# OpenPPL/ppq

Hardware: AMD Instinct MI355X
Metric: calibration samples/sec (RuntimeCalibrationPass, KL 2048-bin, ResNet-50 INT8) (higher is better)
Workload: dtype f32; 1 GPU; ResNet-50 topology (53 Conv + 1 Gemm, BN folded, seeded He init), RuntimeCalibrationPass kl 2048 bins, per-tensor INT8 activations, per-channel INT8 weights, 279 batches x 32 x 3x224x224 per GPU; samples=8928, batch=32, observed_tensors=72, rccl_ranks=1, async_observe=False, cache_params=False, channels_last=False, fuse_params=True, batch_observations=True, reuse_activations=False, replayed_batches=0, hip_graph=auto, graph_replays=0, miopen_find=False

## Files before the change

### ppq_amd/csrc/pointwise_conv.hip

```cpp
#include "common.hpp"
#include "epilogue_sinks.hpp"
#include "job_table.hpp"

namespace ppqhip {
namespace {

typedef float f32x16 __attribute__((ext_vector_type(16)));

struct PwArgs {
    const float* x; const float* w; const float* bias; float* y;
    uint32_t c, o, q;
    uint32_t in_plane, out_plane;
    uint32_t in_w, stride;
    uint32_t tiles_m;
    FastDiv div_plane, div_wo, div_tiles_m;
};

template <int WM, int WN, int TM, int TN, int BK, bool VEC>
__global__ __launch_bounds__(256) void conv1x1_kernel(const PwArgs g) {
    static_assert(WM * WN == 4 && (BK == 16 || BK == 32), "4 waves; BK 16 or 32");
    constexpr int BM = WM * TM * 32, BN = WN * TN * 32, RS = BK + 4, HK = BK / 2, LW = VEC ? 4 : 1;
    constexpr int WL = BM * BK / (256 * LW), XL = BK * BN / (256 * LW);
    constexpr int WROWS = 256 * LW / BK, XROWS = 256 * LW / BN;
    static_assert(BN / LW <= 256 && WL >= 1 && XL >= 1, "tile too small / too wide for the loader");
    typedef float ldv __attribute__((ext_vector_type(LW)));
    __shared__ __attribute__((aligned(16))) float Ws[2][BM * RS];
    __shared__ __attribute__((aligned(16))) float Xs[2][BK * BN];

    const uint32_t t = threadIdx.x, lane = t & 63u, wave = t >> 6;
    const uint32_t tq = fdiv(blockIdx.x, g.div_tiles_m), tm = blockIdx.x - tq * g.tiles_m;
    const uint32_t m0 = tm * BM, q0 = tq * BN;

    const uint32_t wk = (t % (BK / LW)) * LW, wm = t / (BK / LW);
    const uint32_t xc = (t % (BN / LW)) * LW, xk = t / (BN / LW);
    uint32_t woff[WL], xoff;
#pragma unroll
    for (int r = 0; r < WL; r++) woff[r] = min(m0 + wm + WROWS * r, g.o - 1u) * g.c + wk;
    {
        const uint32_t qx = min(q0 + xc, g.q - LW);
        const uint32_t img = fdiv(qx, g.div_plane), p = qx - img * g.out_plane;
        uint32_t src = p;
        if (g.stride != 1u) { const uint32_t oh = fdiv(p, g.div_wo), ow = p - oh * g.div_wo.d; src = (oh * g.in_w + ow) * g.stride; }
        xoff = img * g.c * g.in_plane + src + xk * g.in_plane;
    }
    const uint32_t xstep = XROWS * g.in_plane;
    ldv wr[WL], xr[XL];
    auto load_tile = [&](uint32_t k0) {
        if (k0 + BK <= g.c) {
#pragma unroll
            for (int r = 0; r < WL; r++) wr[r] = *reinterpret_cast<const ldv*>(g.w + (woff[r] + k0));
            const float* xp = g.x + (xoff + k0 * g.in_plane);
#pragma unroll
            for (int r = 0; r < XL; r++) xr[r] = *reinterpret_cast<const ldv*>(xp + r * xstep);
        } else {
#pragma unroll
            for (int r = 0; r < WL; r++) {
                ldv pad = -0.0f;
                wr[r] = (k0 + wk < g.c) ? *reinterpret_cast<const ldv*>(g.w + (woff[r] + k0)) : pad;
            }
#pragma unroll
            for (int r = 0; r < XL; r++) {
                ldv pad = 0.0f;
                xr[r] = (k0 + xk + XROWS * r < g.c) ? *reinterpret_cast<const ldv*>(g.x + (xoff + k0 * g.in_plane + r * xstep)) : pad;
            }
        }
    };
    auto store_tile = [&](int buf) {
#pragma unroll
        for (int r = 0; r < WL; r++) {
            float* row = &Ws[buf][(wm + WROWS * r) * RS];
            if constexpr (VEC) {
                *reinterpret_cast<float2*>(row + (wk >> 1)) = make_float2(wr[r][0], wr[r][2]);
                *reinterpret_cast<float2*>(row + HK + (wk >> 1)) = make_float2(wr[r][1], wr[r][3]);
            } else {
                row[(wk & 1u) * HK + (wk >> 1)] = wr[r][0];
            }
        }
#pragma unroll
        for (int r = 0; r < XL; r++) *reinterpret_cast<ldv*>(&Xs[buf][(xk + XROWS * r) * BN + xc]) = xr[r];
    };

    const uint32_t i = lane & 31u, h = lane >> 5;
    const uint32_t row0 = (wave / WN) * (TM * 32), col0 = (wave % WN) * (TN * 32);
    f32x16 acc[TM][TN];
#pragma unroll
    for (int mt = 0; mt < TM; mt++)
#pragma unroll
        for (int nt = 0; nt < TN; nt++)
#pragma unroll
            for (int r = 0; r < 16; r++) acc[mt][nt][r] = 0.0f;

    const uint32_t tiles_k = (g.c + BK - 1) / BK;
    load_tile(0);
    store_tile(0);
    __syncthreads();
    for (uint32_t kt = 0; kt < tiles_k; kt++) {
        const int buf = (int)(kt & 1u);
        const bool more = kt + 1 < tiles_k;
        if (more) load_tile((kt + 1) * BK);
        const float* ws = &Ws[buf][(row0 + i) * RS + h * HK];
        const float* xs = &Xs[buf][h * BN + col0 + i];
        float a[TM][HK];
#pragma unroll
        for (int mt = 0; mt < TM; mt++)
#pragma unroll
            for (int v = 0; v < HK / 4; v++) {
                const float4 f = *reinterpret_cast<const float4*>(ws + mt * 32 * RS + 4 * v);
                a[mt][4 * v] = f.x; a[mt][4 * v + 1] = f.y; a[mt][4 * v + 2] = f.z; a[mt][4 * v + 3] = f.w;
            }
#pragma unroll
        for (int s = 0; s < HK; s++) {
            float b[TN];
#pragma unroll
            for (int nt = 0; nt < TN; nt++) b[nt] = xs[2 * s * BN + nt * 32];
#pragma unroll
            for (int mt = 0; mt < TM; mt++)
#pragma unroll
                for (int nt = 0; nt < TN; nt++)
                    acc[mt][nt] = __builtin_amdgcn_mfma_f32_32x32x2f32(a[mt][s], b[nt], acc[mt][nt], 0, 0, 0);
        }
        if (more) store_tile(buf ^ 1);
        __syncthreads();
    }

    const bool has_bias = g.bias != nullptr;
    float bv[TM][16];
#pragma unroll
    for (int mt = 0; mt < TM; mt++)
#pragma unroll
        for (int r = 0; r < 16; r++)
            bv[mt][r] = has_bias ? g.bias[min(m0 + row0 + mt * 32 + (r & 3) + 8 * (r >> 2) + 4 * h, g.o - 1u)] : 0.0f;
#pragma unroll
    for (int nt = 0; nt < TN; nt++) {
        const uint32_t qc = q0 + col0 + nt * 32 + i;
        if (qc >= g.q) continue;
        const uint32_t img = fdiv(qc, g.div_plane), p = qc - img * g.out_plane;
        float* yc = g.y + (img * g.o * g.out_plane + p);
#pragma unroll
        for (int mt = 0; mt < TM; mt++)
#pragma unroll
            for (int r = 0; r < 16; r++) {
                const uint32_t row = m0 + row0 + mt * 32 + (r & 3) + 8 * (r >> 2) + 4 * h;
                if (row >= g.o) continue;
                float v = acc[mt][nt][r];
                if (has_bias) v = v + bv[mt][r];
                yc[row * g.out_plane] = v;
            }
    }
}

constexpr int kWM = 2, kWN = 2, kTM = 1, kTN = 1, kBK = 32;

inline bool aligned4(const void* p) { return (reinterpret_cast<uintptr_t>(p) & 3u) == 0; }

struct PwEpArgs {
    const float* bias_b; const float* resid;
    uint32_t tiles, relu;
};

template <int WM, int WN, int BK, bool VEC, int FORM, class SINKS>
__global__ __launch_bounds__(WM * WN * 64, (WM * WN * 64 * kEpStatWgPerCu + 255) / 256)
void conv1x1_epilogue_kernel(const PwArgs g, const PwEpArgs e, const typename SINKS::Args sk) {
    static_assert(BK == 16 || BK == 32, "BK 16 or 32");
    constexpr int NT = WM * WN * 64;
    constexpr bool RESID = FORM != 0, BIAS_B = FORM == 1;
    constexpr int BM = WM * 32, BN = WN * 32, RS = BK + 4, HK = BK / 2, LW = VEC ? 4 : 1;
    constexpr int WL = BM * BK / (NT * LW), XL = BK * BN / (NT * LW);
    constexpr int WROWS = NT * LW / BK, XROWS = NT * LW / BN;
    static_assert(BN / LW <= NT && WL >= 1 && XL >= 1, "tile too small / too wide for the loader");
    typedef float ldv __attribute__((ext_vector_type(LW)));
    __shared__ __attribute__((aligned(16))) float Ws[2][BM * RS];
    __shared__ __attribute__((aligned(16))) float Xs[2][BK * BN];
    __shared__ float Bs[2][2 * BM];
    extern __shared__ int sink_lds[];

    const uint32_t t = threadIdx.x, lane = t & 63u, wave = t >> 6;
    uint32_t tile, tile_end;
    even_split(e.tiles, gridDim.x, blockIdx.x, tile, tile_end);
    SINKS sinks;
    sinks.init(sk, sink_lds);

    const uint32_t wk = (t % (BK / LW)) * LW, wm = t / (BK / LW);
    const uint32_t xc = (t % (BN / LW)) * LW, xk = t / (BN / LW);
    const uint32_t xstep = XROWS * g.in_plane;
    uint32_t m0, q0, woff[WL], xoff;
    float bpre = 0.0f;
    int par = 0;
    auto setup = [&](uint32_t ti) {
        const uint32_t tq = fdiv(ti, g.div_tiles_m), tm = ti - tq * g.tiles_m;
        m0 = tm * BM; q0 = tq * BN;
#pragma unroll
        for (int r = 0; r < WL; r++) woff[r] = min(m0 + wm + WROWS * r, g.o - 1u) * g.c + wk;
        const uint32_t qx = min(q0 + xc, g.q - LW);
        const uint32_t img = fdiv(qx, g.div_plane), p = qx - img * g.out_plane;
        uint32_t src = p;
        if (g.stride != 1u) { const uint32_t oh = fdiv(p, g.div_wo), ow = p - oh * g.div_wo.d; src = (oh * g.in_w + ow) * g.stride; }
        xoff = img * g.c * g.in_plane + src + xk * g.in_plane;
        if (t < 2 * BM) {
            const uint32_t row = min(m0 + (t & (BM - 1)), g.o - 1u);
            bpre = t < BM ? g.bias[row] : (BIAS_B ? e.bias_b[row] : 0.0f);
        }
    };
    ldv wr[WL], xr[XL];
    auto load_tile = [&](uint32_t k0) {
        if (k0 + BK <= g.c) {
#pragma unroll
            for (int r = 0; r < WL; r++) wr[r] = *reinterpret_cast<const ldv*>(g.w + (woff[r] + k0));
            const float* xp = g.x + (xoff + k0 * g.in_plane);
#pragma unroll
            for (int r = 0; r < XL; r++) xr[r] = *reinterpret_cast<const ldv*>(xp + r * xstep);
        } else {
#pragma unroll
            for (int r = 0; r < WL; r++) {
                ldv pad = -0.0f;
                wr[r] = (k0 + wk < g.c) ? *reinterpret_cast<const ldv*>(g.w + (woff[r] + k0)) : pad;
            }
#pragma unroll
            for (int r = 0; r < XL; r++) {
                ldv pad = 0.0f;
                xr[r] = (k0 + xk + XROWS * r < g.c) ? *reinterpret_cast<const ldv*>(g.x + (xoff + k0 * g.in_plane + r * xstep)) : pad;
            }
        }
    };
    auto store_tile = [&](int buf) {
#pragma unroll
        for (int r = 0; r < WL; r++) {
            float* row = &Ws[buf][(wm + WROWS * r) * RS];
            if constexpr (VEC) {
                *reinterpret_cast<float2*>(row + (wk >> 1)) = make_float2(wr[r][0], wr[r][2]);
                *reinterpret_cast<float2*>(row + HK + (wk >> 1)) = make_float2(wr[r][1], wr[r][3]);
            } else {
                row[(wk & 1u) * HK + (wk >> 1)] = wr[r][0];
            }
        }
#pragma unroll
        for (int r = 0; r < XL; r++) *reinterpret_cast<ldv*>(&Xs[buf][(xk + XROWS * r) * BN + xc]) = xr[r];
    };

    const uint32_t i = lane & 31u, h = lane >> 5;
    const uint32_t row0 = (wave / WN) * 32, col0 = (wave % WN) * 32;
    const uint32_t tiles_k = (g.c + BK - 1) / BK;
    const bool relu = e.relu != 0;

    setup(tile);
    load_tile(0);
    sinks.begin();
    for (;;) {
        const uint32_t em0 = m0, eq0 = q0;
        const uint32_t qc = eq0 + col0 + i, rbase = em0 + row0 + 4 * h;
        const bool col_in = qc < g.q;
        const uint32_t qcl = min(qc, g.q - 1u);
        const uint32_t img = fdiv(qcl, g.div_plane), p = qcl - img * g.out_plane;
        const uint32_t ycol = img * g.o * g.out_plane + p;
        f32x16 acc;
#pragma unroll
        for (int r = 0; r < 16; r++) acc[r] = 0.0f;

        auto multiply = [&](int buf) {
            const float* ws = &Ws[buf][(row0 + i) * RS + h * HK];
            const float* xs = &Xs[buf][h * BN + col0 + i];
            float a[HK];
#pragma unroll
            for (int v = 0; v < HK / 4; v++) {
                const float4 f = *reinterpret_cast<const float4*>(ws + 4 * v);
                a[4 * v] = f.x; a[4 * v + 1] = f.y; a[4 * v + 2] = f.z; a[4 * v + 3] = f.w;
            }
#pragma unroll
            for (int s = 0; s < HK; s++) acc = __builtin_amdgcn_mfma_f32_32x32x2f32(a[s], xs[2 * s * BN], acc, 0, 0, 0);
        };
        store_tile(0);
        if (t < 2 * BM) Bs[par][t] = bpre;
        __syncthreads();
        for (uint32_t kt = 0; kt + 1 < tiles_k; kt++) {
            const int buf = (int)(kt & 1u);
            load_tile((kt + 1) * BK);
            multiply(buf);
            store_tile(buf ^ 1);
            __syncthreads();
        }
        float rv[16];
#pragma unroll
        for (int r = 0; r < 16; r++)
            rv[r] = RESID ? e.resid[ycol + min(rbase + (r & 3) + 8 * (r >> 2), g.o - 1u) * g.out_plane] : 0.0f;
        multiply((int)((tiles_k - 1) & 1u));
        __syncthreads();

        const bool next = tile + 1 < tile_end;
        const bool full = em0 + BM <= g.o && eq0 + BN <= g.q;
        const float* bs = &Bs[par][row0 + 4 * h];
#pragma unroll
        for (int j = 0; j < 4; j++) {
            if (j == 2 && next) { setup(tile + 1); load_tile(0); }
            float va[4], vb[4], vo[4], ba[4], bb[4];
#pragma unroll
            for (int u = 0; u < 4; u++) { ba[u] = bs[8 * j + u]; bb[u] = BIAS_B ? bs[BM + 8 * j + u] : 0.0f; }
#pragma unroll
            for (int u = 0; u < 4; u++) {
                const int r = 4 * j + u;
                const float xa = acc[r] + ba[u];
                if (!RESID) { va[u] = act(xa, relu); vb[u] = 0.0f; vo[u] = 0.0f; continue; }
                va[u] = xa;
                float rr = rv[r];
                if (BIAS_B) rr = rr + bb[u];
                vb[u] = rr;
                vo[u] = act(xa + rr, relu);
            }
#pragma unroll
            for (int u = 0; u < 4; u++) {
                const uint32_t row = rbase + u + 8 * j;
                if (col_in && row < g.o) g.y[ycol + min(row, g.o - 1u) * g.out_plane] = RESID ? vo[u] : va[u];
            }
            if (full) {
                EpStored<float4> s4{};
                s4.a = make_float4(va[0], va[1], va[2], va[3]);
                if (BIAS_B) s4.b = make_float4(vb[0], vb[1], vb[2], vb[3]);
                if (RESID) s4.out = make_float4(vo[0], vo[1], vo[2], vo[3]);
                sinks.template feed4<true>(s4, true, j == 0);
            } else {
#pragma unroll
                for (int u = 0; u < 4; u++) {
                    EpStored<float> s1{};
                    s1.a = va[u]; s1.b = vb[u]; s1.out = vo[u];
                    sinks.feed1(s1, col_in && rbase + u + 8 * j < g.o);
                }
            }
            __builtin_amdgcn_sched_barrier(0);
        }
        if (!next) break;
        tile++;
        par ^= 1;
    }
    sinks.finish(sk, blockIdx.x, sink_lds);
}

constexpr int kFWM = 2, kFWN = 4;
static_assert(kFWM * kFWN * 64 == kEpStatBlock, "the fused launch has the sink launches' workgroup");

template <int FORM, class SINKS>
void launch_fused(bool vec, uint32_t grid, uint32_t lds_bytes, hipStream_t s, const PwArgs& g, const PwEpArgs& e,
                  const typename SINKS::Args& sk) {
    if (vec) hipLaunchKernelGGL((conv1x1_epilogue_kernel<kFWM, kFWN, kBK, true, FORM, SINKS>), dim3(grid), dim3(kEpStatBlock), lds_bytes, s, g, e, sk);
    else hipLaunchKernelGGL((conv1x1_epilogue_kernel<kFWM, kFWN, kBK, false, FORM, SINKS>), dim3(grid), dim3(kEpStatBlock), lds_bytes, s, g, e, sk);
}

template <int FORM>
void launch_fused_hist(bool vec, uint32_t grid, hipStream_t s, const PwArgs& g, const PwEpArgs& e, const EpHistSinks& sk, int asym, int clip) {
    constexpr bool R = FORM != 0, B = FORM == 1;
    const uint32_t lds = sk.lds_ints * (uint32_t)sizeof(int);
    switch ((asym ? 2 : 0) | (clip ? 1 : 0)) {
        case 0: launch_fused<FORM, EpHistSet<R, B, false, false, kEpStatBlock, !R>>(vec, grid, lds, s, g, e, sk); break;
        case 1: launch_fused<FORM, EpHistSet<R, B, false, true, kEpStatBlock, !R>>(vec, grid, lds, s, g, e, sk); break;
        case 2: launch_fused<FORM, EpHistSet<R, B, true, false, kEpStatBlock, !R>>(vec, grid, lds, s, g, e, sk); break;
        default: launch_fused<FORM, EpHistSet<R, B, true, true, kEpStatBlock, !R>>(vec, grid, lds, s, g, e, sk); break;
    }
}

int refuse(const char* what, const char* why) {
    set_error("%s: %s", what, why);
    return PPQHIP_ERR_INVALID_VALUE;
}

}
}

using namespace ppqhip;

extern "C" int ppqhip_conv1x1(const float* x, const float* w, const float* bias, float* y, int64_t n, int64_t c, int64_t h, int64_t wd,
                              int64_t o, int64_t stride, void* stream) {
    const char* what = "conv1x1";
    constexpr int64_t kMax = 2147483647;
    if (n < 0 || c <= 0 || h <= 0 || wd <= 0 || o <= 0) { set_error("%s: non-positive size", what); return PPQHIP_ERR_INVALID_VALUE; }
    if (stride != 1 && stride != 2) { set_error("%s: stride must be 1 or 2", what); return PPQHIP_ERR_UNSUPPORTED; }
    if (n == 0) return PPQHIP_OK;
    if (x == nullptr || w == nullptr || y == nullptr) { set_error("%s: null pointer", what); return PPQHIP_ERR_INVALID_VALUE; }
    const int64_t ho = (h - 1) / stride + 1, wo = (wd - 1) / stride + 1;
    if (n > kMax || c > kMax || h > kMax || wd > kMax || o > kMax || (double)n * (double)c * (double)h * (double)wd > (double)kMax
        || (double)n * (double)o * (double)ho * (double)wo > (double)kMax || (double)o * (double)c > (double)kMax) {
        set_error("%s: more than 2^31 - 1 elements in x, w or y", what); return PPQHIP_ERR_INVALID_VALUE;
    }
    std::vector<Span> ins, outs;
    ins.push_back(span_of(x, n * c * h * wd)); ins.push_back(span_of(w, o * c));
    if (bias != nullptr) ins.push_back(span_of(bias, o));
    outs.push_back(span_of(y, n * o * ho * wo));
    if (int st = check_overlap(what, ins, outs)) return st;
    if (!aligned4(x) || !aligned4(w) || !aligned4(y) || !aligned4(bias)) return PPQHIP_NOT_FUSED;

    PwArgs g;
    g.x = x; g.w = w; g.bias = bias; g.y = y;
    g.c = (uint32_t)c; g.o = (uint32_t)o; g.q = (uint32_t)(n * ho * wo);
    g.in_plane = (uint32_t)(h * wd); g.out_plane = (uint32_t)(ho * wo); g.in_w = (uint32_t)wd; g.stride = (uint32_t)stride;
    g.div_plane = make_fastdiv(g.out_plane); g.div_wo = make_fastdiv((uint32_t)wo);
    hipStream_t s = (hipStream_t)stream;
    const bool vec = stride == 1 && g.out_plane % 4u == 0 && c % 4 == 0 && aligned16(x) && aligned16(w);
    constexpr uint32_t BM = kWM * kTM * 32, BN = kWN * kTN * 32;
    g.tiles_m = (g.o + BM - 1) / BM;
    g.div_tiles_m = make_fastdiv(g.tiles_m);
    const dim3 grid(g.tiles_m * ((g.q + BN - 1) / BN));
    if (vec) hipLaunchKernelGGL((conv1x1_kernel<kWM, kWN, kTM, kTN, kBK, true>), grid, dim3(256), 0, s, g);
    else hipLaunchKernelGGL((conv1x1_kernel<kWM, kWN, kTM, kTN, kBK, false>), grid, dim3(256), 0, s, g);
    return finish_launch(what);
}

extern "C" int ppqhip_conv1x1_epilogue(const float* x, const float* w, const float* bias_a, const float* resid, const float* bias_b,
                                       float* out, int64_t n, int64_t c, int64_t h, int64_t wd, int64_t o, int64_t stride, int relu,
                                       int sink_kind, void* dst_a, void* dst_r, void* dst_out, float p0_a, float p1_a, float p0_r,
                                       float p1_r, float p0_out, float p1_out, int64_t num_bins, int asymmetric, int clip_outliers,
                                       int64_t max_workgroups, void* stream) {
    const char* what = "conv1x1_epilogue";
    constexpr int64_t kMax = 2147483647;
    if (n < 0 || c <= 0 || h <= 0 || wd <= 0 || o <= 0) return refuse(what, "non-positive size");
    if (stride != 1 && stride != 2) { set_error("%s: stride must be 1 or 2", what); return PPQHIP_ERR_UNSUPPORTED; }
    if (max_workgroups < 0) return refuse(what, "max_workgroups is negative");
    if (sink_kind != PPQHIP_SINK_NONE && sink_kind != PPQHIP_SINK_MINMAX && sink_kind != PPQHIP_SINK_HIST)
        return refuse(what, "unknown sink kind");
    if (n == 0) return PPQHIP_OK;
    if (x == nullptr || w == nullptr || bias_a == nullptr || out == nullptr) return refuse(what, "null pointer");
    if (resid == nullptr && bias_b != nullptr) return refuse(what, "bias_b without a residual");
    const int64_t ho = (h - 1) / stride + 1, wo = (wd - 1) / stride + 1;
    if (n > kMax || c > kMax || h > kMax || wd > kMax || o > kMax || (double)n * (double)c * (double)h * (double)wd > (double)kMax
        || (double)n * (double)o * (double)ho * (double)wo > (double)kMax || (double)o * (double)c > (double)kMax)
        return refuse(what, "more than 2^31 - 1 elements in x, w or out");
    if (resid == nullptr && (dst_a != nullptr || dst_r != nullptr)) return refuse(what, "without a residual only out has a sink");
    if (bias_b == nullptr && dst_r != nullptr) return refuse(what, "without bias_b, the residual is only read: it has no sink");
    const bool hist = sink_kind == PPQHIP_SINK_HIST, minmax = sink_kind == PPQHIP_SINK_MINMAX;
    if (hist && (num_bins <= 0 || num_bins > kMax)) return refuse(what, "histogram is empty or too large");
    if ((dst_a && (dst_a == dst_r || dst_a == dst_out)) || (dst_r && dst_r == dst_out)) return refuse(what, "two sinks share one accumulator");
    const int64_t ny = n * o * ho * wo;
    std::vector<Span> ins, outs;
    ins.push_back(span_of(x, n * c * h * wd)); ins.push_back(span_of(w, o * c)); ins.push_back(span_of(bias_a, o));
    if (resid != nullptr) ins.push_back(span_of(resid, ny));
    if (bias_b != nullptr) ins.push_back(span_of(bias_b, o));
    outs.push_back(span_of(out, ny));
    if (int st = check_overlap(what, ins, outs)) return st;

    if (!aligned4(x) || !aligned4(w) || !aligned4(bias_a) || !aligned4(resid) || !aligned4(bias_b) || !aligned4(out)) return PPQHIP_NOT_FUSED;
    if (!(minmax || hist) || (dst_a == nullptr && dst_r == nullptr && dst_out == nullptr)) return PPQHIP_NOT_FUSED;
    void* dst[3] = {resid ? dst_a : dst_out, dst_r, resid ? dst_out : nullptr};
    EpMinMaxSinks mm{};
    EpHistSinks hs{};
    if (minmax) for (int k = 0; k < 3; k++) mm.slots[k] = static_cast<float*>(dst[k]);
    if (hist) {
        const float p0[3] = {resid ? p0_a : p0_out, p0_r, p0_out}, p1[3] = {resid ? p1_a : p1_out, p1_r, p1_out};
        hs.bins = (int)num_bins;
        uint64_t ints = 0;
        for (int k = 0; k < 3; k++) {
            hs.rows[k] = static_cast<int*>(dst[k]);
            if (asymmetric) { hs.a0[k] = p0[k]; hs.hs[k] = (p1[k] - p0[k]) / (float)hs.bins; }
            else { hs.a0[k] = 0.f; hs.hs[k] = p0[k]; }
            hs.lds_off[k] = (uint32_t)ints;
            if (hs.rows[k]) ints += (uint64_t)num_bins;
        }
        if (ints > kEpHistLdsInts) return PPQHIP_NOT_FUSED;
        hs.lds_ints = (uint32_t)ints;
    }

    PwArgs g;
    g.x = x; g.w = w; g.bias = bias_a; g.y = out;
    g.c = (uint32_t)c; g.o = (uint32_t)o; g.q = (uint32_t)(n * ho * wo);
    g.in_plane = (uint32_t)(h * wd); g.out_plane = (uint32_t)(ho * wo); g.in_w = (uint32_t)wd; g.stride = (uint32_t)stride;
    g.div_plane = make_fastdiv(g.out_plane); g.div_wo = make_fastdiv((uint32_t)wo);
    const bool vec = stride == 1 && g.out_plane % 4u == 0 && c % 4 == 0 && aligned16(x) && aligned16(w);
    constexpr uint32_t BM = kFWM * 32, BN = kFWN * 32;
    g.tiles_m = (g.o + BM - 1) / BM;
    g.div_tiles_m = make_fastdiv(g.tiles_m);
    PwEpArgs e;
    e.bias_b = bias_b; e.resid = resid; e.relu = relu ? 1u : 0u;
    e.tiles = g.tiles_m * ((g.q + BN - 1) / BN);
    uint32_t grid = (uint32_t)(num_cu() * kEpStatWgPerCu);
    if (grid > e.tiles) grid = e.tiles;
    if (max_workgroups > 0 && (int64_t)grid > max_workgroups) grid = (uint32_t)max_workgroups;
    hipStream_t s = (hipStream_t)stream;
    const int form = resid == nullptr ? 0 : bias_b != nullptr ? 1 : 2;
    if (minmax) {
        const uint32_t lds = 32 * sizeof(float);
        if (form == 0) launch_fused<0, EpMinMaxSet<false, false>>(vec, grid, lds, s, g, e, mm);
        else if (form == 1) launch_fused<1, EpMinMaxSet<true, true>>(vec, grid, lds, s, g, e, mm);
        else launch_fused<2, EpMinMaxSet<true, false>>(vec, grid, lds, s, g, e, mm);
    } else {
        if (form == 0) launch_fused_hist<0>(vec, grid, s, g, e, hs, asymmetric, clip_outliers);
        else if (form == 1) launch_fused_hist<1>(vec, grid, s, g, e, hs, asymmetric, clip_outliers);
        else launch_fused_hist<2>(vec, grid, s, g, e, hs, asymmetric, clip_outliers);
    }
    return finish_launch(what);
}
```

Measured before the change: 4041 samples/s.

## Add two-stage register prefetch pipeline to 1x1 conv kernels for deep channels

Moves the 1x1 conv tile loader and MMA step into a shared PwTile helper. For inputs with at least 512 channels it adds a deeper pipeline that keeps two register stages in flight, prefetching K-tile kt+2 while computing kt. It also unrolls by two with an unguarded full-tile load path. In the fused epilogue kernel the second stage for the next tile is issued during the epilogue, except for one residual/minmax variant. The extra register stage raises VGPR pressure and could lower occupancy, and the plain kernel drops the TM/TN multi-tile template parameters.

```diff
diff --git a/ppq_amd/csrc/pointwise_conv.hip b/ppq_amd/csrc/pointwise_conv.hip
--- a/ppq_amd/csrc/pointwise_conv.hip
+++ b/ppq_amd/csrc/pointwise_conv.hip
@@ -1,3 +1,5 @@
+#include <type_traits>
+
 #include "common.hpp"
 #include "epilogue_sinks.hpp"
 #include "job_table.hpp"
@@ -16,179 +18,28 @@
     FastDiv div_plane, div_wo, div_tiles_m;
 };
 
-template <int WM, int WN, int TM, int TN, int BK, bool VEC>
-__global__ __launch_bounds__(256) void conv1x1_kernel(const PwArgs g) {
-    static_assert(WM * WN == 4 && (BK == 16 || BK == 32), "4 waves; BK 16 or 32");
-    constexpr int BM = WM * TM * 32, BN = WN * TN * 32, RS = BK + 4, HK = BK / 2, LW = VEC ? 4 : 1;
-    constexpr int WL = BM * BK / (256 * LW), XL = BK * BN / (256 * LW);
-    constexpr int WROWS = 256 * LW / BK, XROWS = 256 * LW / BN;
-    static_assert(BN / LW <= 256 && WL >= 1 && XL >= 1, "tile too small / too wide for the loader");
-    typedef float ldv __attribute__((ext_vector_type(LW)));
-    __shared__ __attribute__((aligned(16))) float Ws[2][BM * RS];
-    __shared__ __attribute__((aligned(16))) float Xs[2][BK * BN];
-
-    const uint32_t t = threadIdx.x, lane = t & 63u, wave = t >> 6;
-    const uint32_t tq = fdiv(blockIdx.x, g.div_tiles_m), tm = blockIdx.x - tq * g.tiles_m;
-    const uint32_t m0 = tm * BM, q0 = tq * BN;
-
-    const uint32_t wk = (t % (BK / LW)) * LW, wm = t / (BK / LW);
-    const uint32_t xc = (t % (BN / LW)) * LW, xk = t / (BN / LW);
-    uint32_t woff[WL], xoff;
-#pragma unroll
-    for (int r = 0; r < WL; r++) woff[r] = min(m0 + wm + WROWS * r, g.o - 1u) * g.c + wk;
-    {
-        const uint32_t qx = min(q0 + xc, g.q - LW);
-        const uint32_t img = fdiv(qx, g.div_plane), p = qx - img * g.out_plane;
-        uint32_t src = p;
-        if (g.stride != 1u) { const uint32_t oh = fdiv(p, g.div_wo), ow = p - oh * g.div_wo.d; src = (oh * g.in_w + ow) * g.stride; }
-        xoff = img * g.c * g.in_plane + src + xk * g.in_plane;
-    }
-    const uint32_t xstep = XROWS * g.in_plane;
-    ldv wr[WL], xr[XL];
-    auto load_tile = [&](uint32_t k0) {
-        if (k0 + BK <= g.c) {
-#pragma unroll
-            for (int r = 0; r < WL; r++) wr[r] = *reinterpret_cast<const ldv*>(g.w + (woff[r] + k0));
-            const float* xp = g.x + (xoff + k0 * g.in_plane);
-#pragma unroll
-            for (int r = 0; r < XL; r++) xr[r] = *reinterpret_cast<const ldv*>(xp + r * xstep);
-        } else {
-#pragma unroll
-            for (int r = 0; r < WL; r++) {
-                ldv pad = -0.0f;
-                wr[r] = (k0 + wk < g.c) ? *reinterpret_cast<const ldv*>(g.w + (woff[r] + k0)) : pad;
-            }
-#pragma unroll
-            for (int r = 0; r < XL; r++) {
-                ldv pad = 0.0f;
-                xr[r] = (k0 + xk + XROWS * r < g.c) ? *reinterpret_cast<const ldv*>(g.x + (xoff + k0 * g.in_plane + r * xstep)) : pad;
-            }
-        }
-    };
-    auto store_tile = [&](int buf) {
-#pragma unroll
-        for (int r = 0; r < WL; r++) {
-            float* row = &Ws[buf][(wm + WROWS * r) * RS];
-            if constexpr (VEC) {
-                *reinterpret_cast<float2*>(row + (wk >> 1)) = make_float2(wr[r][0], wr[r][2]);
-                *reinterpret_cast<float2*>(row + HK + (wk >> 1)) = make_float2(wr[r][1], wr[r][3]);
-            } else {
-                row[(wk & 1u) * HK + (wk >> 1)] = wr[r][0];
-            }
-        }
-#pragma unroll
-        for (int r = 0; r < XL; r++) *reinterpret_cast<ldv*>(&Xs[buf][(xk + XROWS * r) * BN + xc]) = xr[r];
-    };
-
-    const uint32_t i = lane & 31u, h = lane >> 5;
-    const uint32_t row0 = (wave / WN) * (TM * 32), col0 = (wave % WN) * (TN * 32);
-    f32x16 acc[TM][TN];
-#pragma unroll
-    for (int mt = 0; mt < TM; mt++)
-#pragma unroll
-        for (int nt = 0; nt < TN; nt++)
-#pragma unroll
-            for (int r = 0; r < 16; r++) acc[mt][nt][r] = 0.0f;
-
-    const uint32_t tiles_k = (g.c + BK - 1) / BK;
-    load_tile(0);
-    store_tile(0);
-    __syncthreads();
-    for (uint32_t kt = 0; kt < tiles_k; kt++) {
-        const int buf = (int)(kt & 1u);
-        const bool more = kt + 1 < tiles_k;
-        if (more) load_tile((kt + 1) * BK);
-        const float* ws = &Ws[buf][(row0 + i) * RS + h * HK];
-        const float* xs = &Xs[buf][h * BN + col0 + i];
-        float a[TM][HK];
-#pragma unroll
-        for (int mt = 0; mt < TM; mt++)
-#pragma unroll
-            for (int v = 0; v < HK / 4; v++) {
-                const float4 f = *reinterpret_cast<const float4*>(ws + mt * 32 * RS + 4 * v);
-                a[mt][4 * v] = f.x; a[mt][4 * v + 1] = f.y; a[mt][4 * v + 2] = f.z; a[mt][4 * v + 3] = f.w;
-            }
-#pragma unroll
-        for (int s = 0; s < HK; s++) {
-            float b[TN];
-#pragma unroll
-            for (int nt = 0; nt < TN; nt++) b[nt] = xs[2 * s * BN + nt * 32];
-#pragma unroll
-            for (int mt = 0; mt < TM; mt++)
-#pragma unroll
-                for (int nt = 0; nt < TN; nt++)
-                    acc[mt][nt] = __builtin_amdgcn_mfma_f32_32x32x2f32(a[mt][s], b[nt], acc[mt][nt], 0, 0, 0);
-        }
-        if (more) store_tile(buf ^ 1);
-        __syncthreads();
-    }
-
-    const bool has_bias = g.bias != nullptr;
-    float bv[TM][16];
-#pragma unroll
-    for (int mt = 0; mt < TM; mt++)
-#pragma unroll
-        for (int r = 0; r < 16; r++)
-            bv[mt][r] = has_bias ? g.bias[min(m0 + row0 + mt * 32 + (r & 3) + 8 * (r >> 2) + 4 * h, g.o - 1u)] : 0.0f;
-#pragma unroll
-    for (int nt = 0; nt < TN; nt++) {
-        const uint32_t qc = q0 + col0 + nt * 32 + i;
-        if (qc >= g.q) continue;
-        const uint32_t img = fdiv(qc, g.div_plane), p = qc - img * g.out_plane;
-        float* yc = g.y + (img * g.o * g.out_plane + p);
-#pragma unroll
-        for (int mt = 0; mt < TM; mt++)
-#pragma unroll
-            for (int r = 0; r < 16; r++) {
-                const uint32_t row = m0 + row0 + mt * 32 + (r & 3) + 8 * (r >> 2) + 4 * h;
-                if (row >= g.o) continue;
-                float v = acc[mt][nt][r];
-                if (has_bias) v = v + bv[mt][r];
-                yc[row * g.out_plane] = v;
-            }
-    }
-}
-
-constexpr int kWM = 2, kWN = 2, kTM = 1, kTN = 1, kBK = 32;
-
-inline bool aligned4(const void* p) { return (reinterpret_cast<uintptr_t>(p) & 3u) == 0; }
-
-struct PwEpArgs {
-    const float* bias_b; const float* resid;
-    uint32_t tiles, relu;
-};
-
-template <int WM, int WN, int BK, bool VEC, int FORM, class SINKS>
-__global__ __launch_bounds__(WM * WN * 64, (WM * WN * 64 * kEpStatWgPerCu + 255) / 256)
-void conv1x1_epilogue_kernel(const PwArgs g, const PwEpArgs e, const typename SINKS::Args sk) {
+template <int BM, int BN, int BK, int NT, bool VEC>
+struct PwTile {
     static_assert(BK == 16 || BK == 32, "BK 16 or 32");
-    constexpr int NT = WM * WN * 64;
-    constexpr bool RESID = FORM != 0, BIAS_B = FORM == 1;
-    constexpr int BM = WM * 32, BN = WN * 32, RS = BK + 4, HK = BK / 2, LW = VEC ? 4 : 1;
-    constexpr int WL = BM * BK / (NT * LW), XL = BK * BN / (NT * LW);
-    constexpr int WROWS = NT * LW / BK, XROWS = NT * LW / BN;
+    static constexpr int RS = BK + 4, HK = BK / 2, LW = VEC ? 4 : 1;
+    static constexpr int WL = BM * BK / (NT * LW), XL = BK * BN / (NT * LW);
+    static constexpr int WROWS = NT * LW / BK, XROWS = NT * LW / BN;
+        static constexpr int WS_FLOATS = 2 * BM * RS, XS_FLOATS = 2 * BK * BN;
     static_assert(BN / LW <= NT && WL >= 1 && XL >= 1, "tile too small / too wide for the loader");
     typedef float ldv __attribute__((ext_vector_type(LW)));
-    __shared__ __attribute__((aligned(16))) float Ws[2][BM * RS];
-    __shared__ __attribute__((aligned(16))) float Xs[2][BK * BN];
-    __shared__ float Bs[2][2 * BM];
-    extern __shared__ int sink_lds[];
-
-    const uint32_t t = threadIdx.x, lane = t & 63u, wave = t >> 6;
-    uint32_t tile, tile_end;
-    even_split(e.tiles, gridDim.x, blockIdx.x, tile, tile_end);
-    SINKS sinks;
-    sinks.init(sk, sink_lds);
-
-    const uint32_t wk = (t % (BK / LW)) * LW, wm = t / (BK / LW);
-    const uint32_t xc = (t % (BN / LW)) * LW, xk = t / (BN / LW);
-    const uint32_t xstep = XROWS * g.in_plane;
-    uint32_t m0, q0, woff[WL], xoff;
-    float bpre = 0.0f;
-    int par = 0;
-    auto setup = [&](uint32_t ti) {
-        const uint32_t tq = fdiv(ti, g.div_tiles_m), tm = ti - tq * g.tiles_m;
-        m0 = tm * BM; q0 = tq * BN;
+    struct Stage { ldv w[WL], x[XL]; };
+
+    float* ws; float* xs;
+    uint32_t wk, wm, xc, xk, xstep;
+    uint32_t woff[WL], xoff;
+
+    __device__ __forceinline__ void init(float* ws_, float* xs_, uint32_t t, const PwArgs& g) {
+        ws = ws_; xs = xs_;
+        wk = (t % (BK / LW)) * LW; wm = t / (BK / LW);
+        xc = (t % (BN / LW)) * LW; xk = t / (BN / LW);
+        xstep = XROWS * g.in_plane;
+    }
+    __device__ __forceinline__ void locate(const PwArgs& g, uint32_t m0, uint32_t q0) {
 #pragma unroll
         for (int r = 0; r < WL; r++) woff[r] = min(m0 + wm + WROWS * r, g.o - 1u) * g.c + wk;
         const uint32_t qx = min(q0 + xc, g.q - LW);
@@ -196,54 +47,191 @@
         uint32_t src = p;
         if (g.stride != 1u) { const uint32_t oh = fdiv(p, g.div_wo), ow = p - oh * g.div_wo.d; src = (oh * g.in_w + ow) * g.stride; }
         xoff = img * g.c * g.in_plane + src + xk * g.in_plane;
+    }
+    template <bool FULL = false>
+    __device__ __forceinline__ void load(const PwArgs& g, Stage& s, uint32_t k0) const {
+        if (FULL || k0 + BK <= g.c) {
+#pragma unroll
+            for (int r = 0; r < WL; r++) s.w[r] = *reinterpret_cast<const ldv*>(g.w + (woff[r] + k0));
+            const float* xp = g.x + (xoff + k0 * g.in_plane);
+#pragma unroll
+            for (int r = 0; r < XL; r++) s.x[r] = *reinterpret_cast<const ldv*>(xp + r * xstep);
+        } else {
+#pragma unroll
+            for (int r = 0; r < WL; r++) {
+                ldv pad = -0.0f;
+                s.w[r] = (k0 + wk < g.c) ? *reinterpret_cast<const ldv*>(g.w + (woff[r] + k0)) : pad;
+            }
+#pragma unroll
+            for (int r = 0; r < XL; r++) {
+                ldv pad = 0.0f;
+                s.x[r] = (k0 + xk + XROWS * r < g.c) ? *reinterpret_cast<const ldv*>(g.x + (xoff + k0 * g.in_plane + r * xstep)) : pad;
+            }
+        }
+    }
+    __device__ __forceinline__ void write(const Stage& s, int buf) const {
+#pragma unroll
+        for (int r = 0; r < WL; r++) {
+            float* row = ws + buf * (BM * RS) + (wm + WROWS * r) * RS;
+            if constexpr (VEC) {
+                *reinterpret_cast<float2*>(row + (wk >> 1)) = make_float2(s.w[r][0], s.w[r][2]);
+                *reinterpret_cast<float2*>(row + HK + (wk >> 1)) = make_float2(s.w[r][1], s.w[r][3]);
+            } else {
+                row[(wk & 1u) * HK + (wk >> 1)] = s.w[r][0];
+            }
+        }
+#pragma unroll
+        for (int r = 0; r < XL; r++) *reinterpret_cast<ldv*>(xs + buf * (BK * BN) + (xk + XROWS * r) * BN + xc) = s.x[r];
+    }
+    __device__ __forceinline__ void multiply(int buf, uint32_t fw, uint32_t fx, f32x16& acc) const {
+        const float* wp = ws + buf * (BM * RS) + fw;
+        const float* xp = xs + buf * (BK * BN) + fx;
+        float a[HK];
+#pragma unroll
+        for (int v = 0; v < HK / 4; v++) {
+            const float4 f = *reinterpret_cast<const float4*>(wp + 4 * v);
+            a[4 * v] = f.x; a[4 * v + 1] = f.y; a[4 * v + 2] = f.z; a[4 * v + 3] = f.w;
+        }
+#pragma unroll
+        for (int s = 0; s < HK; s++) acc = __builtin_amdgcn_mfma_f32_32x32x2f32(a[s], xp[2 * s * BN], acc, 0, 0, 0);
+    }
+    template <int LOAD>
+    __device__ __forceinline__ void step(const PwArgs& g, uint32_t kt, uint32_t tiles_k, Stage& free, Stage& nxt, uint32_t fw, uint32_t fx,
+                                         f32x16& acc) const {
+        if (LOAD > 0) load<true>(g, free, (kt + 2u) * BK);
+        else if (LOAD < 0 && kt + 2u < tiles_k) load(g, free, (kt + 2u) * BK);
+        multiply((int)(kt & 1u), fw, fx, acc);
+        write(nxt, (int)((kt + 1u) & 1u));
+        __syncthreads();
+    }
+    template <class F>
+    __device__ __forceinline__ void steps(const PwArgs& g, uint32_t tiles_k, Stage& s0, Stage& s1, uint32_t fw, uint32_t fx, f32x16& acc,
+                                          F&& staged) const {
+        write(s0, 0);
+        staged();
+        __syncthreads();
+        uint32_t kt = 0;
+        for (; kt + 4u < tiles_k; kt += 2u) { step<1>(g, kt, tiles_k, s0, s1, fw, fx, acc); step<1>(g, kt + 1u, tiles_k, s1, s0, fw, fx, acc); }
+        for (; kt + 2u < tiles_k; kt += 2u) { step<-1>(g, kt, tiles_k, s0, s1, fw, fx, acc); step<-1>(g, kt + 1u, tiles_k, s1, s0, fw, fx, acc); }
+        if (kt + 1u < tiles_k) step<0>(g, kt, tiles_k, s0, s1, fw, fx, acc);
+    }
+    template <class F>
+    __device__ __forceinline__ void steps_shallow(const PwArgs& g, uint32_t tiles_k, Stage& s0, uint32_t fw, uint32_t fx, f32x16& acc,
+                                                  F&& staged) const {
+        write(s0, 0);
+        staged();
+        __syncthreads();
+        for (uint32_t kt = 0; kt + 1u < tiles_k; kt++) {
+            load(g, s0, (kt + 1u) * BK);
+            multiply((int)(kt & 1u), fw, fx, acc);
+            write(s0, (int)((kt + 1u) & 1u));
+            __syncthreads();
+        }
+    }
+};
+
+template <int WM, int WN, int BK, bool VEC, bool DEEP>
+__global__ __launch_bounds__(256) void conv1x1_kernel(const PwArgs g) {
+    static_assert(WM * WN == 4, "4 waves");
+    constexpr int BM = WM * 32, BN = WN * 32;
+    typedef PwTile<BM, BN, BK, 256, VEC> Tile;
+    __shared__ __attribute__((aligned(16))) float Ws[Tile::WS_FLOATS];
+    __shared__ __attribute__((aligned(16))) float Xs[Tile::XS_FLOATS];
+
+    const uint32_t t = threadIdx.x, lane = t & 63u, wave = t >> 6;
+    const uint32_t tq = fdiv(blockIdx.x, g.div_tiles_m), tm = blockIdx.x - tq * g.tiles_m;
+    const uint32_t m0 = tm * BM, q0 = tq * BN;
+
+    Tile tl;
+    tl.init(Ws, Xs, t, g);
+    tl.locate(g, m0, q0);
+    const uint32_t tiles_k = (g.c + BK - 1) / BK;
+    typename Tile::Stage s0, s1;
+    tl.load(g, s0, 0);
+    if (DEEP && 1u < tiles_k) tl.load(g, s1, BK);
+
+    const uint32_t i = lane & 31u, h = lane >> 5;
+    const uint32_t row0 = (wave / WN) * 32, col0 = (wave % WN) * 32;
+    const uint32_t fw = (row0 + i) * Tile::RS + h * Tile::HK, fx = h * BN + col0 + i;
+    f32x16 acc;
+#pragma unroll
+    for (int r = 0; r < 16; r++) acc[r] = 0.0f;
+
+    if (DEEP) tl.steps(g, tiles_k, s0, s1, fw, fx, acc, [] {});
+    else tl.steps_shallow(g, tiles_k, s0, fw, fx, acc, [] {});
+    tl.multiply((int)((tiles_k - 1) & 1u), fw, fx, acc);
+
+    const bool has_bias = g.bias != nullptr;
+    float bv[16];
+#pragma unroll
+    for (int r = 0; r < 16; r++) bv[r] = has_bias ? g.bias[min(m0 + row0 + (r & 3) + 8 * (r >> 2) + 4 * h, g.o - 1u)] : 0.0f;
+    const uint32_t qc = q0 + col0 + i;
+    if (qc >= g.q) return;
+    const uint32_t img = fdiv(qc, g.div_plane), p = qc - img * g.out_plane;
+    float* yc = g.y + (img * g.o * g.out_plane + p);
+#pragma unroll
+    for (int r = 0; r < 16; r++) {
+        const uint32_t row = m0 + row0 + (r & 3) + 8 * (r >> 2) + 4 * h;
+        if (row >= g.o) continue;
+        float v = acc[r];
+        if (has_bias) v = v + bv[r];
+        yc[row * g.out_plane] = v;
+    }
+}
+
+constexpr int kWM = 2, kWN = 2, kBK = 32;
+constexpr uint32_t kPwDeepFrom = 512;
+
+inline bool aligned4(const void* p) { return (reinterpret_cast<uintptr_t>(p) & 3u) == 0; }
+
+struct PwEpArgs {
+    const float* bias_b; const float* resid;
+    uint32_t tiles, relu;
+};
+
+template <int WM, int WN, int BK, bool VEC, bool DEEP, int FORM, class SINKS>
+__global__ __launch_bounds__(WM * WN * 64, (WM * WN * 64 * kEpStatWgPerCu + 255) / 256)
+void conv1x1_epilogue_kernel(const PwArgs g, const PwEpArgs e, const typename SINKS::Args sk) {
+    constexpr int NT = WM * WN * 64;
+    constexpr bool RESID = FORM != 0, BIAS_B = FORM == 1;
+    constexpr int BM = WM * 32, BN = WN * 32;
+    typedef PwTile<BM, BN, BK, NT, VEC> Tile;
+    __shared__ __attribute__((aligned(16))) float Ws[Tile::WS_FLOATS];
+    __shared__ __attribute__((aligned(16))) float Xs[Tile::XS_FLOATS];
+    __shared__ float Bs[2][2 * BM];
+    extern __shared__ int sink_lds[];
+
+    const uint32_t t = threadIdx.x, lane = t & 63u, wave = t >> 6;
+    uint32_t tile, tile_end;
+    even_split(e.tiles, gridDim.x, blockIdx.x, tile, tile_end);
+    SINKS sinks;
+    sinks.init(sk, sink_lds);
+
+    Tile tl;
+    tl.init(Ws, Xs, t, g);
+    uint32_t m0, q0;
+    float bpre = 0.0f;
+    int par = 0;
+    auto setup = [&](uint32_t ti) {
+        const uint32_t tq = fdiv(ti, g.div_tiles_m), tm = ti - tq * g.tiles_m;
+        m0 = tm * BM; q0 = tq * BN;
+        tl.locate(g, m0, q0);
         if (t < 2 * BM) {
             const uint32_t row = min(m0 + (t & (BM - 1)), g.o - 1u);
             bpre = t < BM ? g.bias[row] : (BIAS_B ? e.bias_b[row] : 0.0f);
         }
     };
-    ldv wr[WL], xr[XL];
-    auto load_tile = [&](uint32_t k0) {
-        if (k0 + BK <= g.c) {
-#pragma unroll
-            for (int r = 0; r < WL; r++) wr[r] = *reinterpret_cast<const ldv*>(g.w + (woff[r] + k0));
-            const float* xp = g.x + (xoff + k0 * g.in_plane);
-#pragma unroll
-            for (int r = 0; r < XL; r++) xr[r] = *reinterpret_cast<const ldv*>(xp + r * xstep);
-        } else {
-#pragma unroll
-            for (int r = 0; r < WL; r++) {
-                ldv pad = -0.0f;
-                wr[r] = (k0 + wk < g.c) ? *reinterpret_cast<const ldv*>(g.w + (woff[r] + k0)) : pad;
-            }
-#pragma unroll
-            for (int r = 0; r < XL; r++) {
-                ldv pad = 0.0f;
-                xr[r] = (k0 + xk + XROWS * r < g.c) ? *reinterpret_cast<const ldv*>(g.x + (xoff + k0 * g.in_plane + r * xstep)) : pad;
-            }
-        }
-    };
-    auto store_tile = [&](int buf) {
-#pragma unroll
-        for (int r = 0; r < WL; r++) {
-            float* row = &Ws[buf][(wm + WROWS * r) * RS];
-            if constexpr (VEC) {
-                *reinterpret_cast<float2*>(row + (wk >> 1)) = make_float2(wr[r][0], wr[r][2]);
-                *reinterpret_cast<float2*>(row + HK + (wk >> 1)) = make_float2(wr[r][1], wr[r][3]);
-            } else {
-                row[(wk & 1u) * HK + (wk >> 1)] = wr[r][0];
-            }
-        }
-#pragma unroll
-        for (int r = 0; r < XL; r++) *reinterpret_cast<ldv*>(&Xs[buf][(xk + XROWS * r) * BN + xc]) = xr[r];
-    };
+    typename Tile::Stage st0, st1;
 
     const uint32_t i = lane & 31u, h = lane >> 5;
     const uint32_t row0 = (wave / WN) * 32, col0 = (wave % WN) * 32;
     const uint32_t tiles_k = (g.c + BK - 1) / BK;
     const bool relu = e.relu != 0;
 
+    const uint32_t fw = (row0 + i) * Tile::RS + h * Tile::HK, fx = h * BN + col0 + i;
     setup(tile);
-    load_tile(0);
+    tl.load(g, st0, 0);
+    if (DEEP && 1u < tiles_k) tl.load(g, st1, BK);
     sinks.begin();
     for (;;) {
         const uint32_t em0 = m0, eq0 = q0;
@@ -256,33 +244,14 @@
 #pragma unroll
         for (int r = 0; r < 16; r++) acc[r] = 0.0f;
 
-        auto multiply = [&](int buf) {
-            const float* ws = &Ws[buf][(row0 + i) * RS + h * HK];
-            const float* xs = &Xs[buf][h * BN + col0 + i];
-            float a[HK];
-#pragma unroll
-            for (int v = 0; v < HK / 4; v++) {
-                const float4 f = *reinterpret_cast<const float4*>(ws + 4 * v);
-                a[4 * v] = f.x; a[4 * v + 1] = f.y; a[4 * v + 2] = f.z; a[4 * v + 3] = f.w;
-            }
-#pragma unroll
-            for (int s = 0; s < HK; s++) acc = __builtin_amdgcn_mfma_f32_32x32x2f32(a[s], xs[2 * s * BN], acc, 0, 0, 0);
-        };
-        store_tile(0);
-        if (t < 2 * BM) Bs[par][t] = bpre;
-        __syncthreads();
-        for (uint32_t kt = 0; kt + 1 < tiles_k; kt++) {
-            const int buf = (int)(kt & 1u);
-            load_tile((kt + 1) * BK);
-            multiply(buf);
-            store_tile(buf ^ 1);
-            __syncthreads();
-        }
+        auto staged = [&] { if (t < 2 * BM) Bs[par][t] = bpre; };
+        if (DEEP) tl.steps(g, tiles_k, st0, st1, fw, fx, acc, staged);
+        else tl.steps_shallow(g, tiles_k, st0, fw, fx, acc, staged);
         float rv[16];
 #pragma unroll
         for (int r = 0; r < 16; r++)
             rv[r] = RESID ? e.resid[ycol + min(rbase + (r & 3) + 8 * (r >> 2), g.o - 1u) * g.out_plane] : 0.0f;
-        multiply((int)((tiles_k - 1) & 1u));
+        tl.multiply((int)((tiles_k - 1) & 1u), fw, fx, acc);
         __syncthreads();
 
         const bool next = tile + 1 < tile_end;
@@ -290,7 +259,8 @@
         const float* bs = &Bs[par][row0 + 4 * h];
 #pragma unroll
         for (int j = 0; j < 4; j++) {
-            if (j == 2 && next) { setup(tile + 1); load_tile(0); }
+            if (j == 2 && next) { setup(tile + 1); tl.load(g, st0, 0); }
+            if (DEEP && !RESID && j == 3 && next && 1u < tiles_k) tl.load(g, st1, BK);
             float va[4], vb[4], vo[4], ba[4], bb[4];
 #pragma unroll
             for (int u = 0; u < 4; u++) { ba[u] = bs[8 * j + u]; bb[u] = BIAS_B ? bs[BM + 8 * j + u] : 0.0f; }
@@ -327,6 +297,7 @@
             __builtin_amdgcn_sched_barrier(0);
         }
         if (!next) break;
+        if (DEEP && RESID && 1u < tiles_k) tl.load(g, st1, BK);
         tile++;
         par ^= 1;
     }
@@ -339,8 +310,14 @@
 template <int FORM, class SINKS>
 void launch_fused(bool vec, uint32_t grid, uint32_t lds_bytes, hipStream_t s, const PwArgs& g, const PwEpArgs& e,
                   const typename SINKS::Args& sk) {
-    if (vec) hipLaunchKernelGGL((conv1x1_epilogue_kernel<kFWM, kFWN, kBK, true, FORM, SINKS>), dim3(grid), dim3(kEpStatBlock), lds_bytes, s, g, e, sk);
-    else hipLaunchKernelGGL((conv1x1_epilogue_kernel<kFWM, kFWN, kBK, false, FORM, SINKS>), dim3(grid), dim3(kEpStatBlock), lds_bytes, s, g, e, sk);
+    const dim3 gd(grid), bd(kEpStatBlock);
+    constexpr bool kDeepVec = !(FORM == 1 && std::is_same<SINKS, EpMinMaxSet<true, true>>::value);
+    switch ((vec ? 2 : 0) | (g.c >= kPwDeepFrom ? 1 : 0)) {
+        case 3: hipLaunchKernelGGL((conv1x1_epilogue_kernel<kFWM, kFWN, kBK, true, kDeepVec, FORM, SINKS>), gd, bd, lds_bytes, s, g, e, sk); break;
+        case 2: hipLaunchKernelGGL((conv1x1_epilogue_kernel<kFWM, kFWN, kBK, true, false, FORM, SINKS>), gd, bd, lds_bytes, s, g, e, sk); break;
+        case 1: hipLaunchKernelGGL((conv1x1_epilogue_kernel<kFWM, kFWN, kBK, false, true, FORM, SINKS>), gd, bd, lds_bytes, s, g, e, sk); break;
+        default: hipLaunchKernelGGL((conv1x1_epilogue_kernel<kFWM, kFWN, kBK, false, false, FORM, SINKS>), gd, bd, lds_bytes, s, g, e, sk); break;
+    }
 }
 
 template <int FORM>
@@ -392,12 +369,16 @@
     g.div_plane = make_fastdiv(g.out_plane); g.div_wo = make_fastdiv((uint32_t)wo);
     hipStream_t s = (hipStream_t)stream;
     const bool vec = stride == 1 && g.out_plane % 4u == 0 && c % 4 == 0 && aligned16(x) && aligned16(w);
-    constexpr uint32_t BM = kWM * kTM * 32, BN = kWN * kTN * 32;
+    constexpr uint32_t BM = kWM * 32, BN = kWN * 32;
     g.tiles_m = (g.o + BM - 1) / BM;
     g.div_tiles_m = make_fastdiv(g.tiles_m);
     const dim3 grid(g.tiles_m * ((g.q + BN - 1) / BN));
-    if (vec) hipLaunchKernelGGL((conv1x1_kernel<kWM, kWN, kTM, kTN, kBK, true>), grid, dim3(256), 0, s, g);
-    else hipLaunchKernelGGL((conv1x1_kernel<kWM, kWN, kTM, kTN, kBK, false>), grid, dim3(256), 0, s, g);
+    switch ((vec ? 2 : 0) | (g.c >= kPwDeepFrom ? 1 : 0)) {
+        case 3: hipLaunchKernelGGL((conv1x1_kernel<kWM, kWN, kBK, true, true>), grid, dim3(256), 0, s, g); break;
+        case 2: hipLaunchKernelGGL((conv1x1_kernel<kWM, kWN, kBK, true, false>), grid, dim3(256), 0, s, g); break;
+        case 1: hipLaunchKernelGGL((conv1x1_kernel<kWM, kWN, kBK, false, true>), grid, dim3(256), 0, s, g); break;
+        default: hipLaunchKernelGGL((conv1x1_kernel<kWM, kWN, kBK, false, false>), grid, dim3(256), 0, s, g); break;
+    }
     return finish_launch(what);
 }
 
```

New measurement: 4063 samples/s, median of 6. Within noise of the previous version (+0.5%).
